# SixLabors/ZlibStream

Measured on AMD Instinct MI355X. Metric: deflate MB/s (input) at level 6, 64 MiB buffers, higher is better.
Workload: dtype u8; 1 GPU; english64: 1 x 67108864-byte pseudo-random-English (Zipf words of alice29.txt) buffer per GPU, level 6, zlib framing, inputs resident in HBM; level=6, buffer_bytes=67108864, buffers_per_gpu=1, compressed_bytes=27425826, parallelism=independent buffers, 1 GPU(s), no collective in the data path

## Files before the change

### zlibstream_amd/csrc/zs_device.h

```cpp
#pragma once
#include <cstddef>
#include "zs_core.h"
#include "zs_lit_engine.h"
#include "zs_fast_sweep.h"
#include "zs_rle.h"

namespace zs {

constexpr int kMatchTile = 16384;
constexpr int kMatchBack = 32512;
constexpr int kMatchFwd = 272;
constexpr int kMatchLdsBytes = kMatchBack + kMatchTile + kMatchFwd;
constexpr int kMatchLdsLinks = kMatchBack + kMatchTile;
constexpr int kMatchLds = kMatchLdsBytes + 2 * kMatchLdsLinks;
constexpr int kAdlerPiece = 65536;

constexpr int64_t kScratchWindow = 0;
constexpr int64_t kScratchHead = 66560;
constexpr int64_t kScratchPrev = kScratchHead + 2 * kHashSize;
constexpr int64_t kScratchHead32 = kScratchPrev + 2 * kWSize;
constexpr int64_t kScratchBytes = kScratchHead32 + 4 * kHashSize;

struct StreamDesc {
    const uint8_t *in;
// ... 78 lines not shown
    uint32_t nsyms;
    int32_t nblocks;
    int64_t out_len;
    uint32_t adler;
    int32_t status;
    int64_t end_bits;
    int32_t r_seg, r_slot, r_kfired, r_kslot;
    uint32_t r_total;
    int32_t r_ncut;
    int32_t r_cut_e[8], r_cut_done[8];
    int32_t deferred, r_scan;
    int32_t r_cutidx;
    int32_t nc[2], cuts_same, cut_diff_idx, cut_diff_pos;
    int32_t poison;
    int32_t spec_run_tiles, spec_ok, spec_wrong;
};
constexpr uint32_t kSpecBail = 1u << 30;
ZS_HD uint32_t spec_pack(int guess, int exit_slot, int count, bool bail) {
    return (uint32_t)guess | ((uint32_t)exit_slot << 9) | ((uint32_t)count << 18) | (bail ? kSpecBail : 0u);
}
ZS_HD int spec_guess(uint32_t r) { return (int)(r & 0x1FF); }
ZS_HD int spec_exit(uint32_t r) { return (int)((r >> 9) & 0x1FF); }
ZS_HD int spec_count(uint32_t r) { return (int)((r >> 18) & 0xFFF); }
constexpr int kSpecMinInput = 1 << 20;
constexpr int kSpecLenBits = 10;
constexpr int kSpecWarm = 128;
constexpr int kSpecRunsDen = 8;
struct K5Spec {
    uint32_t *rec;
    uint32_t *base;
// ... 33 lines not shown
```

### zlibstream_amd/csrc/zs_engine.hip

```cpp
#include <hip/hip_runtime.h>

#include <algorithm>
#include <cstdio>
#include <cstdlib>
#include <cstring>
#include <functional>
#include <string>
#include <thread>
#include <vector>

#define ZS_BUILDING_LIBRARY
#include "../../include/zsgpu.h"
#include "zs_kernels.hip"
#include "zs_inflate_par.hip"
#include "zs_inflate_tok.hip"
#include "zs_png.hip"
#include "zs_crc32.hip"
#include "zs_gzip.hip"
#include "zs_zip.hip"
#include "zs_tiff.hip"
#include "zs_exr.hip"
#include "zs_plan.h"

using namespace zs;

namespace {

struct DevBuf {
    void *p = nullptr;
    size_t cap = 0;
};

enum Stage {
    kStClear, kStAdler, kStLinks, kStMatch, kStChunkMap, kStSegMap, kStResolve, kStExpand, kStEmitSyms, kStTail, kStTrees,
    kStOffsets, kStEmitBits, kStSpecWalk, kStSpecVerify, kStCrc32, kStSpecCompact, kStPngExpand, kStPngSplit, kStPngPack, kStPngSurvey, kStPngCompose, kStPngDiff, kStPngCrop, kStCount
};
const char *const kStageNames[kStCount] = {"clear", "adler", "links", "match", "chunkmap", "segmap", "resolve", "expand",
                                           "emit_syms", "tail", "trees", "offsets", "emit_bits", "spec_walk", "spec_verify", "crc32_frame",
                                           "spec_compact", "png_expand", "png_split", "png_pack", "png_survey", "png_compose", "png_diff", "png_crop"};

enum PngBuf {
    kBufPngImg, kBufPngSeg, kBufPngCtr, kBufPngFimg, kBufPngScratch, kBufPngA7img, kBufPngInflated, kBufPngPasses, kBufCrcDesc, kBufCrcRes, kBufPngZs, kBufPngGather,
    kBufPngXimg, kBufPngRaw, kBufPngSimg, kBufPngSplit, kBufPngGimg, kBufPngVimg, kBufPngVrec, kBufPngPacked, kBufPngCimg, kBufPngFrames, kBufPngDimg, kBufPngDrec,
    kBufPngKimg, kBufPngCrop,
    kBufWrapHead, kBufWrapGather, kBufWrapZs, kBufWrapFiles, kBufZipZs, kBufTiffChunks, kBufTiffDesc, kBufTiffZs, kBufExrChunks, kBufExrDesc, kBufExrZs, kBufExrSegs,
    kBufPngCount
};

struct PlanCache;

}

struct zs_ctx {
    int device = 0;
    hipStream_t stream = nullptr;
    hipStream_t aux = nullptr;
    hipEvent_t ev_fork = nullptr, ev_join = nullptr, ev_pre0 = nullptr, ev_pre = nullptr;
    hipEvent_t ev_spec[4] = {};
    std::string err;
    bool profiling = false;
    int fast_fallbacks = 0;
    int round_runs = 0;
    int cut_rounds = 0;
    int lit_fallbacks = 0;
    int spec_streams = 0, spec_fallbacks = 0, spec_wrong_chunks = 0;
    int spec_periodic = 0;
    int64_t dbg_blk_off = 0, dbg_chunk_off = 0, dbg_nchunks = 0, dbg_spec_n = 0, dbg_n_spec = 0;
    int64_t lit_engine_bytes = 0;
    std::vector<int64_t> inf_used;
    int64_t *inf_probe = nullptr;
    int inf_lane_streams = 0;
    int inf_wave_streams = 0;
    int64_t png_segments = 0;
// ... 97 lines not shown
template <class T>
T *dev(DevBuf &b) {
    return (T *)b.p;
}


struct RunOpts : PlanRun {
    int64_t end_bits = 0;
};

struct LaunchEnv {
    bool no_plan_reuse = getenv("ZS_NO_PLAN_REUSE") != nullptr, no_supmap = getenv("ZS_NO_SUPMAP") != nullptr;
    bool no_defer = getenv("ZS_NO_DEFER") != nullptr, force_rounds = getenv("ZS_FORCE_ROUNDS") != nullptr;
    bool tail_serial = getenv("ZS_TAIL_SERIAL") != nullptr, tail_fork = getenv("ZS_TAIL_FORK") != nullptr, fast_no_probe = getenv("ZS_FAST_NO_PROBE") != nullptr;
    bool no_whole_runs = getenv("ZS_NO_WHOLE_RUNS") != nullptr, whole_runs = getenv("ZS_WHOLE_RUNS") != nullptr;
    bool debug = getenv("ZS_DEBUG") != nullptr, debug_cuts = getenv("ZS_DEBUG_CUTS") != nullptr, debug_fa = getenv("ZS_DEBUG_FA") != nullptr;
    const char *debug_chain = getenv("ZS_DEBUG_CHAIN"), *debug_chain_want = getenv("ZS_DEBUG_CHAIN_WANT");
    int k5_ahead = getenv("ZS_K5_AHEAD") ? atoi(getenv("ZS_K5_AHEAD")) : 1;
    int spec_corrupt = getenv("ZS_SPEC_CORRUPT") ? atoi(getenv("ZS_SPEC_CORRUPT")) : -1;
    static bool host_times() {
        static const bool v = getenv("ZS_HOST_TIMES") != nullptr;
        return v;
    }
    static const char *eb_tiles() {
        static const char *const v = getenv("ZS_EB_TILES");
        return v;
    }
};
struct RoundsEnv {
    int max_rounds = getenv("ZS_FR_MAX_ROUNDS") ? atoi(getenv("ZS_FR_MAX_ROUNDS")) : 0;
// ... 34 lines not shown
    PlanEnv penv = plan_env_read();
    LaunchEnv env;
    FoldedWrites folded;
    PlanArgs pa;
    bool any_writes = false, no_rounds_this_call = false, plan_hit = false, plan_keep = false;
    double ht_plan = 0, ht_launched = 0;
    const StreamDesc *d_sd = nullptr;
    StreamState *d_st = nullptr, *hst = nullptr;
    const uint2 *d_work = nullptr;
    bool prof = false;
    K5Spec k5s{};
    int spec_ok_streams = 0;
    bool need_maps = true, spec_ran = false;
    bool fork_recorded = false;
    bool tail_late = false, tail_serial = false, use_sup = false;
    int defer_mode = 0, cut_stride = 0;
    bool done = false, answer = false;

    double ht_us() const { return std::chrono::duration<double, std::micro>(std::chrono::steady_clock::now() - ht0).count(); }
    const uint2 *work(int list) const { return d_work + lay.work[list]; }
    void mark(int i) {
        if (prof) (void)hipEventRecord(c->ev[i], stream);
    }
    bool rerun(int force_seq_, bool rounds_, const std::vector<uint8_t> *force_lit_) {
        c->lit_engine_bytes -= pl.lit_bytes;
        done = true;
        return answer = run_pipeline(c, n, in, in_len, out, out_cap, out_len, status, level, strategy, hash_variant, stream, writes, force_seq_, ro, rounds_, force_lit_);
    }
    void launch_tail(hipStream_t on) {
        hipLaunchKernelGGL(zs_tail_kernel, dim3((unsigned)n), dim3(1024), kTailLds, on, d_sd, d_st, dev<uint16_t>(c->link),
// ... 431 lines not shown
        for (int s0 = 0; s0 < n; s0 += 65535) launch(dim3((unsigned)((max_tiles + 3) / 4), (unsigned)std::min(n - s0, 65535)), s0);
    };
    tiles([&](dim3 tg, int s0) { hipLaunchKernelGGL(zs_rle_starts_kernel, tg, dim3(256), 0, stream, d_sd, rt, s0); });
    hipLaunchKernelGGL(zs_rle_scan_kernel, dim3((unsigned)n), dim3(1024), 0, stream, d_sd, rt);
    tiles([&](dim3 tg, int s0) {
        hipLaunchKernelGGL(zs_rle_pass_kernel<0>, tg, dim3(256), 0, stream, d_sd, rt, dev<uint32_t>(c->syms), dev<int32_t>(c->blk_end), dev<int32_t>(c->blk_top), s0);
    });
    hipLaunchKernelGGL(zs_rle_sums_kernel, dim3((unsigned)n), dim3(1024), 0, stream, d_sd, d_st, rt);
    tiles([&](dim3 tg, int s0) {
        hipLaunchKernelGGL(zs_rle_pass_kernel<1>, tg, dim3(256), 0, stream, d_sd, rt, dev<uint32_t>(c->syms), dev<int32_t>(c->blk_end), dev<int32_t>(c->blk_top), s0);
    });
    return true;
}

bool DeflateCall::tails_and_symbols() {
    if (!tail_late && !tail_serial) {
        if (!fork_recorded || need_maps) ZS_HIP(c, hipEventRecord(c->ev_fork, stream));
        ZS_HIP(c, hipStreamWaitEvent(c->aux, c->ev_fork, 0));
        launch_tail(c->aux);
        ZS_HIP(c, hipEventRecord(c->ev_join, c->aux));
    }
    if (!pl.w_segs.empty() && need_maps)
        hipLaunchKernelGGL(zs_expand_kernel, dim3((unsigned)((pl.w_segs.size() + 63) / 64)), dim3(64), 0, stream, d_sd, d_st,
                           work(kWSegs), (int)pl.w_segs.size(), dev<uint2>(c->mm), dev<uint16_t>(c->link),
                           dev<uint32_t>(c->maps), dev<uint16_t>(c->seg_entry), dev<uint32_t>(c->seg_symbase),
                           dev<uint8_t>(c->stale), dev<uint16_t>(c->entry), dev<uint32_t>(c->symbase), c->crc_tab, lv, strategy,
                           hash_variant);
    mark(8);
    if (!pl.w_chunks.empty() && need_maps)
        hipLaunchKernelGGL((zs_emit_syms_lane_kernel<4, 0>), dim3((unsigned)((pl.w_chunks.size() + 63) / 64)), dim3(kK5Threads), 0, stream, d_sd, d_st,
                           work(kWChunks), (int)pl.w_chunks.size(), dev<uint2>(c->mm), dev<uint16_t>(c->link), dev<uint16_t>(c->entry),
                           dev<uint32_t>(c->symbase), dev<uint32_t>(c->syms), dev<int32_t>(c->blk_end), dev<int32_t>(c->blk_top),
                           c->crc_tab, lv, strategy, hash_variant, env.k5_ahead, k5s);
    mark(9);
    if (tail_serial) launch_tail(stream);
    else if (!tail_late) ZS_HIP(c, hipStreamWaitEvent(stream, c->ev_join, 0));
    hipLaunchKernelGGL(zs_body_blocks_kernel, dim3((unsigned)n), dim3(256), 0, stream, d_sd, d_st, dev<int32_t>(c->blk_end),
                       dev<int32_t>(c->blk_top), dev<BlockRec>(c->blocks), dev<uint32_t>(c->syms));
    if (tail_late) launch_tail(stream);
    return true;
}

bool DeflateCall::spec_runs() {
    if (!env.fast_no_probe && force_seq == 0 && !pl.any_dual) {
        hipLaunchKernelGGL(zs_fast_probe_kernel, dim3((unsigned)n), dim3(256), 0, stream, d_sd, dev<uint16_t>(c->link), dev<int32_t>(c->run_fail));
        std::vector<int32_t> np((size_t)n, 0);
        ZS_HIP(c, hipMemcpyAsync(np.data(), c->run_fail.p, 4 * (size_t)n, hipMemcpyDeviceToHost, stream));
        ZS_HIP(c, hipStreamSynchronize(stream));
        for (int i = 0; i < n; i++)
            if (np[(size_t)i]) {
                ZS_HIP(c, hipStreamSynchronize(c->aux));
                return rerun(1, false, force_lit);
            }
// ... 40 lines not shown
                       dev<uint32_t>(c->run_syms), dev<FastRunOut>(c->run_outs), dev<uint32_t>(c->syms), dev<int32_t>(c->blk_end),
                       dev<int32_t>(c->blk_top));
    hipLaunchKernelGGL(zs_fast_blocks_kernel, dim3((unsigned)n), dim3(64), 0, stream, d_sd, d_st, dev<FastRunOut>(c->run_outs),
                       dev<int32_t>(c->blk_end), dev<int32_t>(c->blk_top), dev<BlockRec>(c->blocks), n);
    return true;
}

bool DeflateCall::blocks_and_bits() {
    const int trees_threads = pl.w_blocks.size() > 8192 ? 128 : 256;
    if (n >= 64 && !penv.no_live_list) {
        int32_t *const d_live = (int32_t *)((uint8_t *)c->sd.p + lay.sd_bytes);
        hipLaunchKernelGGL(zs_live_scan_kernel, dim3(1), dim3(1024), 0, stream, d_st, n, d_live);
        hipLaunchKernelGGL(zs_live_fill_kernel, dim3((unsigned)((pl.w_blocks.size() + 255) / 256)), dim3(256), 0, stream, d_live, n,
                           (uint32_t)pl.w_blocks.size(), dev<uint2>(c->work) + lay.work[kWBlocks]);
    }
    hipLaunchKernelGGL(zs_trees_kernel, dim3((unsigned)pl.w_blocks.size()), dim3(trees_threads), 0, stream, d_sd, d_st, work(kWBlocks),
                       dev<uint32_t>(c->syms), dev<BlockRec>(c->blocks), dev<TreeWork>(c->trees), dev<BlockInfo>(c->info), dev<int32_t>(c->tile_bits), strategy, level);
    mark(11);
    ZS_HIP(c, hipStreamWaitEvent(stream, c->ev_pre, 0));
    hipLaunchKernelGGL(zs_offsets_kernel, dim3((unsigned)n), dim3(256), 0, stream, d_sd, d_st, dev<BlockRec>(c->blocks),
                       dev<BlockInfo>(c->info), dev<TreeWork>(c->trees), dev<uint32_t>(c->pieces), level, n);
    mark(12);
    int eb_tiles = kEbTiles;
    if (level != 0) {
        int64_t longest = 0;
        for (int i = 0; i < n; i++) longest = std::max(longest, in_len[i]);
        eb_tiles = (int)std::min<int64_t>(kEbTiles, (longest + 1) / kEbTile + 1);
    }
    if (env.eb_tiles()) eb_tiles = std::max(1, std::min(kEbTiles, atoi(env.eb_tiles())));
    hipLaunchKernelGGL(zs_emit_bits_kernel, dim3((unsigned)pl.w_blocks.size(), (unsigned)(1 + eb_tiles)), dim3(256), 0, stream, d_sd, d_st,
                       work(kWBlocks), dev<uint32_t>(c->syms), dev<BlockRec>(c->blocks), dev<TreeWork>(c->trees), dev<BlockInfo>(c->info),
                       dev<int32_t>(c->tile_bits));
    mark(13);
    ZS_HIP(c, hipGetLastError());
    hst = (StreamState *)c->pinned;
    ZS_HIP(c, hipMemcpyAsync(hst, d_st, sizeof(StreamState) * (size_t)n, hipMemcpyDeviceToHost, stream));
    ht_launched = ht_us();
    ZS_HIP(c, hipStreamSynchronize(stream));
    pc.in_flight = false;
    if (pc.valid && !plan_hit) pc.gen = c->plan_gen;
    if (env.host_times())
        fprintf(stderr, "zs: host: plan + uploads %.0f us%s, all launched at %.0f us, device done at %.0f us\n", ht_plan, c->plan_reused ? " (kept plan)" : "", ht_launched,
                ht_us());
    c->last_op = lv.func == 1 ? 2 : 0;
    return true;
}

void DeflateCall::debug_dumps() {
// ... 21 lines not shown
        const size_t nw = wr->ends.size();
        std::vector<int32_t> wb(nw);
        (void)hipMemcpy(wb.data(), pl.sd[0].wr_blk, 4 * nw, hipMemcpyDeviceToHost);
        fprintf(stderr, "[zs] run of %lld bytes, %zu Writes, %d blocks, body ends at %d, resume %d; blocks before each Write:", (long long)in_len[0], nw, hst[0].nblocks,
                pl.sd[0].body_end, pl.sd[0].resume);
        for (size_t k = 0; k < nw && k < 24; k++) fprintf(stderr, " %d(end %lld, flush %d)", wb[k], (long long)wr->ends[k], wr->flush.empty() ? 0 : wr->flush[k]);
        fprintf(stderr, "\n");
    }
}

void DeflateCall::stage_times() {
    for (int i = 0; i < kStCount; i++) {
        float ms = 0;
        if (i >= kStLinks && i <= kStEmitBits) (void)hipEventElapsedTime(&ms, c->ev[i], c->ev[i + 1]);
        c->stage_ms[i] = ms;
    }
    if (spec_ran) {
        float a = 0, b = 0, m = 0;
        (void)hipEventElapsedTime(&a, c->ev[kStChunkMap], c->ev_spec[0]);
        (void)hipEventElapsedTime(&b, c->ev_spec[0], c->ev_spec[1]);
        (void)hipEventElapsedTime(&m, c->ev_spec[1], c->ev[kStChunkMap + 1]);
        c->stage_ms[kStSpecWalk] = a, c->stage_ms[kStSpecVerify] = b, c->stage_ms[kStChunkMap] = m;
        float k = 0;
        (void)hipEventElapsedTime(&k, c->ev_spec[2], c->ev_spec[3]);
        c->stage_ms[kStSpecCompact] = k;
        c->stage_ms[kStSpecVerify] = b > k ? b - k : 0;
    }
}

bool DeflateCall::finish() {
// ... 145 lines not shown
void zs_ctx_destroy(zs_ctx *c);
int zs_ctx_create(int device, zs_ctx **out) {
    if (!out) return ZS_STREAM_ERROR;
    *out = nullptr;
    int count = 0;
    if (hipGetDeviceCount(&count) != hipSuccess || count <= 0 || device < 0 || device >= count) return ZS_STREAM_ERROR;
    if (hipSetDevice(device) != hipSuccess) return ZS_STREAM_ERROR;
    zs_ctx *c = new zs_ctx();
    c->device = device;
    if (hipStreamCreateWithFlags(&c->stream, hipStreamNonBlocking) != hipSuccess) {
        zs_ctx_destroy(c);
        return ZS_MEM_ERROR;
    }
    for (auto &e : c->ev) (void)hipEventCreate(&e);
    for (auto &e : c->ev_spec) (void)hipEventCreate(&e);
    for (auto &e : c->ev_png) (void)hipEventCreate(&e);
    {
        int *d_ok = nullptr, ok = 0;
        if (hipMalloc((void **)&d_ok, sizeof(int)) != hipSuccess) {
            zs_ctx_destroy(c);
            return ZS_MEM_ERROR;
        }
        hipLaunchKernelGGL(zs_lds_order_kernel, dim3(1), dim3(64), 0, c->stream, d_ok);
        const bool copied = hipMemcpyAsync(&ok, d_ok, sizeof(int), hipMemcpyDeviceToHost, c->stream) == hipSuccess &&
                            hipStreamSynchronize(c->stream) == hipSuccess;
        (void)hipFree(d_ok);
        if (!copied || !ok) {
            fprintf(stderr, "zsgpu: LDS lane-order self-test failed on device %d; this build cannot run there\n", device);
            zs_ctx_destroy(c);
            return ZS_STREAM_ERROR;
        }
    }
    if (hipStreamCreateWithFlags(&c->aux, hipStreamNonBlocking) != hipSuccess ||
        hipEventCreateWithFlags(&c->ev_fork, hipEventDisableTiming) != hipSuccess ||
        hipEventCreateWithFlags(&c->ev_join, hipEventDisableTiming) != hipSuccess ||
        hipEventCreateWithFlags(&c->ev_pre0, hipEventDisableTiming) != hipSuccess ||
        hipEventCreateWithFlags(&c->ev_pre, hipEventDisableTiming) != hipSuccess ||
        hipEventCreateWithFlags(&c->ev_verdict, hipEventDisableTiming) != hipSuccess) {
        zs_ctx_destroy(c);
        return ZS_MEM_ERROR;
    }
    std::vector<uint32_t> tab(1024);
    for (int t = 0; t < 4; t++)
        for (int i = 0; i < 256; i++) tab[(size_t)t * 256 + i] = crc32c_table_entry(t, (uint32_t)i);
    if (hipMalloc((void **)&c->crc_tab, 4096) != hipSuccess ||
        hipMemcpy(c->crc_tab, tab.data(), 4096, hipMemcpyHostToDevice) != hipSuccess ||
        hipFuncSetAttribute((const void *)zs_match_kernel, hipFuncAttributeMaxDynamicSharedMemorySize, kMatchLds + 16) != hipSuccess ||
        hipFuncSetAttribute((const void *)zs_resolve_kernel, hipFuncAttributeMaxDynamicSharedMemorySize, kResolveLds) != hipSuccess ||
        hipFuncSetAttribute((const void *)zs_links_kernel, hipFuncAttributeMaxDynamicSharedMemorySize, kLkLds) != hipSuccess ||
        hipFuncSetAttribute((const void *)zs_tail_kernel, hipFuncAttributeMaxDynamicSharedMemorySize, kTailLds) != hipSuccess ||
        hipFuncSetAttribute((const void *)zs_fast_run_kernel, hipFuncAttributeMaxDynamicSharedMemorySize, kFastRunLds) != hipSuccess ||
        hipFuncSetAttribute((const void *)zs_fast_sweep_kernel<1024, kFsTile1, false>, hipFuncAttributeMaxDynamicSharedMemorySize, (fs_lds_bytes<1024, kFsTile1>())) != hipSuccess ||
// ... 36 lines not shown
        if (e) (void)hipEventDestroy(e);
    if (c->pinned) (void)hipHostFree(c->pinned);
    if (c->plan_pin) (void)hipHostFree(c->plan_pin);
    delete c->plan;
    if (c->ev_verdict) (void)hipEventDestroy(c->ev_verdict);
    if (c->pin_io) (void)hipHostFree(c->pin_io);
    if (c->pin_out) (void)hipHostFree(c->pin_out);
    for (auto &e : c->ev)
        if (e) (void)hipEventDestroy(e);
    for (auto &e : c->ev_spec)
        if (e) (void)hipEventDestroy(e);
    if (c->ev_fork) (void)hipEventDestroy(c->ev_fork);
    if (c->ev_join) (void)hipEventDestroy(c->ev_join);
    if (c->ev_pre0) (void)hipEventDestroy(c->ev_pre0);
    if (c->ev_pre) (void)hipEventDestroy(c->ev_pre);
    if (c->aux) (void)hipStreamDestroy(c->aux);
    if (c->stream) (void)hipStreamDestroy(c->stream);
    delete c;
}

const char *zs_ctx_last_error(const zs_ctx *c) { return c ? c->err.c_str() : "no context"; }

int64_t zs_deflate_bound(int64_t n) { return n + (n >> 3) + 1024; }

void zs_ctx_set_profiling(zs_ctx *c, int enable) {
    if (c) c->profiling = enable != 0;
}
int zs_ctx_stage_count(const zs_ctx *) { return kStCount; }
int64_t zs_ctx_counter(const zs_ctx *c, const char *name) {
    if (!c || !name) return -1;
// ... 29 lines not shown
        memcpy(out, state, sizeof state);
        return sizeof state;
    }
    if (k == "blk_end") src = dev<int32_t>(c->blk_end) + c->dbg_blk_off, bytes = 4 * (int64_t)(ss.body_syms / kBlockSyms);
    else if (k == "blk_top") src = dev<int32_t>(c->blk_top) + c->dbg_blk_off, bytes = 4 * (int64_t)(ss.body_syms / kBlockSyms);
    else if (k == "symbase") src = dev<uint32_t>(c->symbase) + c->dbg_chunk_off, bytes = 4 * c->dbg_nchunks;
    else if (k == "spec_base") src = dev<uint32_t>(c->spec_rec) + c->dbg_n_spec, bytes = 4 * c->dbg_spec_n;
    else return -1;
    if (bytes > cap || (bytes > 0 && !src)) return -1;
    if (bytes > 0 && hipMemcpy(out, src, (size_t)bytes, hipMemcpyDeviceToHost) != hipSuccess) return -1;
    return bytes;
}

const char *zs_ctx_stage_name(const zs_ctx *c, int s) {
    static const char *const inf_names[6] = {"inf_find", "inf_measure", "inf_chain", "inf_decode", "inf_windows", "inf_resolve"};
    if (s == kStCrc32 || s == kStSpecCompact || s == kStPngExpand || s == kStPngSplit || s == kStPngPack || s == kStPngSurvey || s == kStPngCompose || s == kStPngDiff || s == kStPngCrop) return kStageNames[s];
    if (c && c->last_op == 1) return s >= 0 && s < 6 ? inf_names[s] : "";
    if (c && c->last_op == 2 && s == kStExpand) return "fast_sweep";
    if (c && c->last_op == 2 && s == kStTail) return "fast_runs+tail";
    return s >= 0 && s < kStCount ? kStageNames[s] : "";
}
double zs_ctx_stage_ms(const zs_ctx *c, int s) { return c && s >= 0 && s < kStCount ? c->stage_ms[s] : 0.0; }

int zs_deflate_batch_device(zs_ctx *c, int n, const void *const *in, const int64_t *in_len, void *const *out,
                            const int64_t *out_cap, int64_t *out_len, int *status, int level, int strategy, int hash_variant,
                            void *hip_stream) {
    if (!check_args(c, n, in_len, level, strategy)) return ZS_STREAM_ERROR;
    if (n == 0) return ZS_OK;
    if (hipSetDevice(c->device) != hipSuccess) return ZS_STREAM_ERROR;
    hipStream_t s = hip_stream ? (hipStream_t)hip_stream : c->stream;
    int rc = ZS_OK;
// ... 746 lines not shown
```

### zlibstream_amd/csrc/zs_kernels.hip

```cpp
#include <hip/hip_runtime.h>

#include <type_traits>

#include "zs_device.h"
#include "zs_png.h"

namespace zs {

typedef uint32_t __attribute__((aligned(1))) u32u;
typedef uint64_t __attribute__((aligned(1))) u64u;
typedef const __attribute__((address_space(1))) uint8_t *gcbytes;
typedef __attribute__((address_space(1))) uint8_t *gbytes_w;
__device__ __forceinline__ gcbytes as_global(const uint8_t *p) { return (gcbytes)(uintptr_t)p; }
__device__ __forceinline__ gbytes_w as_global(uint8_t *p) { return (gbytes_w)(uintptr_t)p; }
typedef const __attribute__((address_space(1))) uint32_t __attribute__((aligned(1))) *gcu32u;
typedef const __attribute__((address_space(1))) uint64_t __attribute__((aligned(1))) *gcu64u;
__device__ __forceinline__ uint32_t g_u32_bytes(gcbytes p) {
    return (uint32_t)p[0] | ((uint32_t)p[1] << 8) | ((uint32_t)p[2] << 16) | ((uint32_t)p[3] << 24);
}
typedef uint32_t u32x4 __attribute__((ext_vector_type(4)));
typedef const __attribute__((address_space(1))) u32x4 *gcu32x4;
__device__ __forceinline__ uint32_t lds_u32(const uint8_t *base, int idx) {
    const uint32_t *q = (const uint32_t *)(base + (idx & ~3));
    return __builtin_amdgcn_alignbyte(q[1], q[0], (uint32_t)idx & 3u);
// ... 1977 lines not shown
        out[i] = v;
        before += i < cut ? sym_len(v) : 0;
    }
    if (cut < 0) return;
#pragma unroll
    for (int d = 32; d >= 1; d >>= 1) before += __shfl_xor(before, d, 64);
    if (lane != 0) return;
    const ChunkCtx cx = spec_chunk_ctx(s, c, sp.len_bits);
    const int64_t start = spec_first_start(cx.cs, spec_guess(r)) + before;
    const bool odd = cx.m != 0 && slab[sp.stride - 1] == (uint32_t)cut;
    const uint32_t bi = (base + (uint32_t)cut) / kBlockSyms;
    blk_end[s.blk_off + bi] = (int32_t)spec_sym_end(start, slab[cut]);
    blk_top[s.blk_off + bi] = (int32_t)spec_sym_top(start, odd);
}

__global__ __launch_bounds__(256) void zs_body_blocks_kernel(const StreamDesc *sd, const StreamState *st, const int32_t *blk_end,
                                                             const int32_t *blk_top, BlockRec *blocks, uint32_t *syms) {
    const StreamDesc s = sd[blockIdx.x];
    if (s.fast_runs > 0 || st[blockIdx.x].deferred) return;
    if (s.resume)
        for (uint32_t i = threadIdx.x; i < s.start_syms; i += blockDim.x) syms[s.sym_off + i] = s.persist->syms[i];
    const int nb_body = (int)(st[blockIdx.x].body_syms / kBlockSyms);
    BlockRec *blk = blocks + s.blk_off;
    for (int i = threadIdx.x; i < nb_body; i += blockDim.x) {
        int64_t start = i ? blk_end[s.blk_off + i - 1] : (s.resume ? s.start_block : 0);
        int64_t end = blk_end[s.blk_off + i];
        BlockRec r;
        r.start = start;
        r.sym_start = (int64_t)i * kBlockSyms;
        r.stored_len = (int32_t)(end - start);
        r.nsyms = kBlockSyms;
        r.can_store = start >= s.base0 + (int64_t)kWSize * (s.rle_end >= 0 ? rle_refills_fired_at(blk_top[s.blk_off + i], s.kl)
                                                                            : refills_fired_at(blk_top[s.blk_off + i] - s.base0, s.kl));
        r.eof = 0;
        blk[i] = r;
    }
    if (s.wr_blk && s.wr_end && s.n_wr > 1) {
        const StreamState &ss = st[blockIdx.x];
        const int64_t read_to = s.nsegs > 0 ? (int64_t)s.seg_after[ss.k_done] : 0;
        for (int w = 1 + (int)threadIdx.x; w < s.n_wr; w += blockDim.x) {
            if (s.wr_end[w - 1] >= read_to) continue;
            const int64_t bound = s.wr_end[w - 1] - (kMinLookahead - 1);
            int lo = 0, hi = nb_body;
            while (lo < hi) {
                const int mid = (lo + hi) >> 1;
                if ((int64_t)blk_top[s.blk_off + mid] < bound) lo = mid + 1;
                else hi = mid;
            }
            s.wr_blk[w] = lo;
        }
    }
// ... 711 lines not shown
        if (live_pre[mid] <= (int32_t)g) lo = mid;
        else hi = mid - 1;
    }
    work[g] = make_uint2((uint32_t)lo, g - (uint32_t)live_pre[lo]);
}

#ifdef ZS_BS_PROF
#define BS_PF(i) { const long long now_ = wall_clock64(); pf[i] += now_ - pf_t; pf_t = now_; }
#else
#define BS_PF(i)
#endif
typedef u32x4 __attribute__((aligned(4))) u32x4a4;
typedef u32x4 __attribute__((aligned(8))) u32x4a8;
__global__ __launch_bounds__(256) void zs_trees_kernel(const StreamDesc *sd, const StreamState *st, const uint2 *work,
                                                       const uint32_t *syms, const BlockRec *blocks, TreeWork *trees,
                                                       BlockInfo *info, int32_t *tile_bits, int strategy, int level) {
    __shared__ __attribute__((aligned(16))) TreeWork tw;
    __shared__ SideTree sw;
    __shared__ uint32_t hl[kLCodes], hd[kDCodes];
    __shared__ uint32_t hk[kHeapSize + 8];
    __shared__ uint32_t pd[kHeapSize + 1], nc[16];
    __shared__ uint32_t hk2[SideTree::kHeap + 8], pd2[SideTree::kHeap + 1], nc2[16];
    __shared__ uint32_t sh_tile[2 * kEbTiles];
    __shared__ int sh_type;
#ifdef ZS_BS_PROF
    long long pf[8] = {0, 0, 0, 0, 0, 0, 0, 0}, pf_t = wall_clock64();
#endif
    uint2 w = work[blockIdx.x];
    if (w.x == kNoWork || st[w.x].deferred) return;
    const StreamDesc s = sd[w.x];
    const int b = (int)w.y;
    if (b >= st[w.x].nblocks) return;
    const BlockRec r = blocks[s.blk_off + b];
    if (level == 0 && r.nsyms == 0 && s.plan_nblk > 0) {
        if (threadIdx.x == 0) {
            BlockInfo bi;
            bi.type = r.can_store ? 0 : 1;
            bi.bits = r.can_store ? 0 : 10;
            bi.bit_start = 0;
            info[s.blk_off + b] = bi;
        }
        return;
    }
    const int tid = (int)threadIdx.x, nthr = (int)blockDim.x, lane = tid & 63, wave = tid >> 6;
    for (int i = tid; i < kLCodes; i += nthr) hl[i] = 0;
    for (int i = tid; i < kDCodes; i += nthr) hd[i] = 0;
    if (tid < 2 * kEbTiles) sh_tile[tid] = 0;
// ... 146 lines not shown
    if (w0) atomicOr(w, w0);
    if (w1) atomicOr(w + 1, w1);
    if (w2) atomicOr(w + 2, w2);
}
struct OrBitsAt {
    uint8_t *out;
    int64_t cap;
    int64_t bit_base;
    __device__ void operator()(int64_t pos, uint32_t v, int nbits) const {
        pos -= bit_base;
        if ((pos >> 3) + 12 <= cap) or_bits(out, pos, v, nbits);
    }
};
__global__ __launch_bounds__(256) void zs_offsets_kernel(const StreamDesc *sd, StreamState *st, const BlockRec *blocks,
                                                         BlockInfo *info, const TreeWork *trees, const uint32_t *adler_pieces,
                                                         int level, int nstreams) {
    __shared__ int32_t sh_type[1024], sh_bits[1024], sh_len[1024], sh_eof[1024];
    __shared__ int64_t sh_start[1024];
    __shared__ uint32_t ad_v[256];
    __shared__ uint64_t ad_len[256];
    __shared__ int64_t sh_pos, sh_wsum[4];
    __shared__ int sh_bad;
    FlushAcct fa;
    int fa_w = 0;
    const bool flushing = sd[blockIdx.x].wr_flush != nullptr;
    const int si = blockIdx.x;
    if (st[si].deferred) return;
    const StreamDesc s = sd[si];
    StreamState &ss = st[si];
    const int nb = ss.nblocks;
    LitPersist *ps = s.persist;
    const int64_t start_bits = s.cont_bits ? ps->fa.bits : 16;
    const int64_t bit_base = s.cont_bits ? (start_bits & ~7LL) : 0;
    if (threadIdx.x == 0) sh_pos = start_bits, sh_bad = 0;
    const OrBitsAt fa_put{s.out, s.out_cap, bit_base};
    if (flushing) {
        if (s.cont_bits) fa = ps->fa;
        else fa_init(fa, s.out_chunk, level, s.raw != 0);
        if (!s.mid_write) fa_enter(fa);
    }
    if (threadIdx.x == 0 && s.cont_bits && s.out_cap > 0) s.out[0] = (uint8_t)s.carry_byte;
    __syncthreads();
    for (int b0 = 0; b0 < nb; b0 += 1024) {
        int cnt = nb - b0 < 1024 ? nb - b0 : 1024;
        for (int i = threadIdx.x; i < cnt; i += 256) {
            const BlockInfo bi = info[s.blk_off + b0 + i];
            const BlockRec r = blocks[s.blk_off + b0 + i];
            sh_type[i] = bi.type, sh_bits[i] = bi.bits, sh_len[i] = r.stored_len, sh_eof[i] = r.eof;
        }
        __syncthreads();
        int irregular = 0;
        for (int i = threadIdx.x; i < cnt; i += 256) irregular |= (sh_type[i] == 0) || (sh_eof[i] && i != cnt - 1);
        irregular = __syncthreads_or(irregular | (int)flushing);
        if (!irregular) {
            const int lane = threadIdx.x & 63, wave = threadIdx.x >> 6;
            int64_t b4[4], mine = 0;
            for (int k = 0; k < 4; k++) {
                const int i = threadIdx.x * 4 + k;
// ... 39 lines not shown
                if (flushing) {
                    fa.bits = pos;
                    fa.last_eob_len = sh_type[i] == 0 ? 8 : sh_type[i] == 1 ? 7 : trees[s.blk_off + b0 + i].ltree[kEndBlock].dl;
                    const int f = sh_eof[i] >> 1;
                    if (f) fa_end_of_write(fa, f, fa_put);
                    else fa_after_block(fa);
                    pos = fa.bits;
                }
            }
            sh_pos = pos;
        }
        __syncthreads();
        for (int i = threadIdx.x; i < cnt; i += 256) info[s.blk_off + b0 + i].bit_start = sh_start[i] - bit_base;
        __syncthreads();
    }
    uint32_t acc = 1;
    uint64_t acc_len = 0;
    {
        const int per = (s.n_adler + 255) / 256;
        for (int k = 0; k < per; k++) {
            int i = threadIdx.x * per + k;
            if (i >= s.n_adler) break;
            int64_t len = (int64_t)s.n - (int64_t)i * kAdlerPiece;
            if (len > kAdlerPiece) len = kAdlerPiece;
            acc = adler_combine(acc, adler_pieces[s.adler_off + i], (uint64_t)len);
            acc_len += (uint64_t)len;
        }
        ad_v[threadIdx.x] = acc, ad_len[threadIdx.x] = acc_len;
    }
    __syncthreads();
// ... 15 lines not shown
        ss.out_len = bytes;
        ss.status = sh_bad ? -2 : (bytes + 8 > s.out_cap ? -5 : 0);
        return;
    }
    int64_t total = (pos - bit_base) / 8 + 4;
    ss.out_len = total;
    if (sh_bad) {
        ss.status = -2;
        return;
    }
    if (total > s.out_cap) {
        ss.status = -5;
        return;
    }
    ss.status = 0;
    if (!s.cont_bits) {
        unsigned hdr = zlib_header(level);
        s.out[0] = (uint8_t)(hdr >> 8);
        s.out[1] = (uint8_t)hdr;
    }
    uint8_t *t = s.out + (pos - bit_base) / 8;
    t[0] = (uint8_t)(ad >> 24), t[1] = (uint8_t)(ad >> 16), t[2] = (uint8_t)(ad >> 8), t[3] = (uint8_t)ad;
}

struct OrPut {
    uint8_t *out;
    int64_t pos;
    __device__ void operator()(unsigned value, int nbits) {
        or_bits(out, pos, value, nbits);
        pos += nbits;
    }
// ... 19 lines not shown
        const uint32_t w0 = (uint32_t)lo, w1 = (uint32_t)(lo >> 32), w2 = sh ? (uint32_t)(v >> (64 - sh)) : 0;
        if (w0) atomicOr(&w[k], w0);
        if (w1) atomicOr(&w[k + 1], w1);
        if (w2) atomicOr(&w[k + 2], w2);
        pos += (uint32_t)nbits;
    }
    __device__ void operator()(unsigned value, int nbits) { put64(value, nbits); }
};
#ifdef ZS_BS_PROF
#define BS_PF(i) { const long long now_ = wall_clock64(); pf[i] += now_ - pf_t; pf_t = now_; }
#else
#define BS_PF(i)
#endif
__global__ __launch_bounds__(256) void zs_emit_bits_kernel(const StreamDesc *sd, const StreamState *st, const uint2 *work,
                                                           const uint32_t *syms, const BlockRec *blocks, const TreeWork *trees,
                                                           const BlockInfo *info, const int32_t *tile_bits) {
    __shared__ uint32_t lt[kLCodes], dt[kDCodes];
    __shared__ uint32_t obuf[kEbWords];
    __shared__ uint32_t wsum[4];
    __shared__ uint32_t sh_bits;
#ifdef ZS_BS_PROF
    long long pf[4] = {0, 0, 0, 0}, pf_t = wall_clock64();
#endif
    uint2 w = work[blockIdx.x];
    if (w.x == kNoWork || st[w.x].deferred) return;
    const StreamDesc s = sd[w.x];
    const int b = (int)w.y;
    if (b >= st[w.x].nblocks || st[w.x].status != 0) return;
    const BlockRec r = blocks[s.blk_off + b];
    const BlockInfo bi = info[s.blk_off + b];
    uint8_t *out = s.out;
    const int tid = threadIdx.x, lane = lane_id(), wave = tid >> 6;
    const int part = (int)blockIdx.y, ntl = (int)gridDim.y - 1;
    if (bi.type == 0) {
        int64_t pos = bi.bit_start;
        int64_t byte = (pos + 3 + 7) >> 3;
        if (part == 0 && tid == 0) {
            or_bits(out, pos, (uint64_t)(r.eof & 1), 3);
            unsigned len = (unsigned)r.stored_len;
            out[byte] = (uint8_t)len, out[byte + 1] = (uint8_t)(len >> 8);
            out[byte + 2] = (uint8_t)~len, out[byte + 3] = (uint8_t)(~len >> 8);
        }
        const gcbytes src = as_global(s.in) + (r.start - s.abs_off);
        const gbytes_w dst = as_global(out) + byte + 4;
        typedef u32x4 __attribute__((aligned(1))) u32x4u;
// ... 367 lines not shown
```

Baseline: 15870 MB/s.

## Split deflate backend into body and tail parts overlapped across two streams

```diff
diff --git a/zlibstream_amd/csrc/zs_device.h b/zlibstream_amd/csrc/zs_device.h
--- a/zlibstream_amd/csrc/zs_device.h
+++ b/zlibstream_amd/csrc/zs_device.h
@@ -116,6 +116,8 @@
     int32_t nc[2], cuts_same, cut_diff_idx, cut_diff_pos;
     int32_t poison;
     int32_t spec_run_tiles, spec_ok, spec_wrong;
+    int32_t body_bad;
+    int64_t body_bits;
 };
 constexpr uint32_t kSpecBail = 1u << 30;
 ZS_HD uint32_t spec_pack(int guess, int exit_slot, int count, bool bail) {
diff --git a/zlibstream_amd/csrc/zs_engine.hip b/zlibstream_amd/csrc/zs_engine.hip
--- a/zlibstream_amd/csrc/zs_engine.hip
+++ b/zlibstream_amd/csrc/zs_engine.hip
@@ -33,11 +33,11 @@
 
 enum Stage {
     kStClear, kStAdler, kStLinks, kStMatch, kStChunkMap, kStSegMap, kStResolve, kStExpand, kStEmitSyms, kStTail, kStTrees,
-    kStOffsets, kStEmitBits, kStSpecWalk, kStSpecVerify, kStCrc32, kStSpecCompact, kStPngExpand, kStPngSplit, kStPngPack, kStPngSurvey, kStPngCompose, kStPngDiff, kStPngCrop, kStCount
+    kStOffsets, kStEmitBits, kStSpecWalk, kStSpecVerify, kStCrc32, kStSpecCompact, kStPngExpand, kStPngSplit, kStPngPack, kStPngSurvey, kStPngCompose, kStPngDiff, kStPngCrop, kStPart1, kStCount
 };
 const char *const kStageNames[kStCount] = {"clear", "adler", "links", "match", "chunkmap", "segmap", "resolve", "expand",
                                            "emit_syms", "tail", "trees", "offsets", "emit_bits", "spec_walk", "spec_verify", "crc32_frame",
-                                           "spec_compact", "png_expand", "png_split", "png_pack", "png_survey", "png_compose", "png_diff", "png_crop"};
+                                           "spec_compact", "png_expand", "png_split", "png_pack", "png_survey", "png_compose", "png_diff", "png_crop", "part1_chain"};
 
 enum PngBuf {
     kBufPngImg, kBufPngSeg, kBufPngCtr, kBufPngFimg, kBufPngScratch, kBufPngA7img, kBufPngInflated, kBufPngPasses, kBufCrcDesc, kBufCrcRes, kBufPngZs, kBufPngGather,
@@ -57,6 +57,7 @@
     hipStream_t aux = nullptr;
     hipEvent_t ev_fork = nullptr, ev_join = nullptr, ev_pre0 = nullptr, ev_pre = nullptr;
     hipEvent_t ev_spec[4] = {};
+    hipEvent_t ev_syms = nullptr, ev_part0 = nullptr, ev_part1[2] = {};
     std::string err;
     bool profiling = false;
     int fast_fallbacks = 0;
@@ -184,6 +185,7 @@
     bool no_defer = getenv("ZS_NO_DEFER") != nullptr, force_rounds = getenv("ZS_FORCE_ROUNDS") != nullptr;
     bool tail_serial = getenv("ZS_TAIL_SERIAL") != nullptr, tail_fork = getenv("ZS_TAIL_FORK") != nullptr, fast_no_probe = getenv("ZS_FAST_NO_PROBE") != nullptr;
     bool no_whole_runs = getenv("ZS_NO_WHOLE_RUNS") != nullptr, whole_runs = getenv("ZS_WHOLE_RUNS") != nullptr;
+    bool no_split_backend = getenv("ZS_NO_SPLIT_BACKEND") != nullptr;
     bool debug = getenv("ZS_DEBUG") != nullptr, debug_cuts = getenv("ZS_DEBUG_CUTS") != nullptr, debug_fa = getenv("ZS_DEBUG_FA") != nullptr;
     const char *debug_chain = getenv("ZS_DEBUG_CHAIN"), *debug_chain_want = getenv("ZS_DEBUG_CHAIN_WANT");
     int k5_ahead = getenv("ZS_K5_AHEAD") ? atoi(getenv("ZS_K5_AHEAD")) : 1;
@@ -248,6 +250,7 @@
     bool need_maps = true, spec_ran = false;
     bool fork_recorded = false;
     bool tail_late = false, tail_serial = false, use_sup = false;
+    bool split = false;
     int defer_mode = 0, cut_stride = 0;
     bool done = false, answer = false;
 
@@ -709,11 +712,18 @@
 }
 
 bool DeflateCall::tails_and_symbols() {
+    const bool beside_k5 = need_maps && (!pl.w_segs.empty() || !pl.w_chunks.empty());
+    if (!tail_late && !tail_serial && (n < 64 || penv.no_live_list) && !env.no_split_backend && pl.n_runs == 0 && !beside_k5) {
+        int64_t longest = 0;
+        for (int i = 0; i < n; i++) longest = std::max(longest, in_len[i]);
+        split = longest >= kBlockSyms;
+    }
     if (!tail_late && !tail_serial) {
         if (!fork_recorded || need_maps) ZS_HIP(c, hipEventRecord(c->ev_fork, stream));
         ZS_HIP(c, hipStreamWaitEvent(c->aux, c->ev_fork, 0));
         launch_tail(c->aux);
-        ZS_HIP(c, hipEventRecord(c->ev_join, c->aux));
+        if (split && prof) (void)hipEventRecord(c->ev_part1[0], c->aux);
+        if (!split) ZS_HIP(c, hipEventRecord(c->ev_join, c->aux));
     }
     if (!pl.w_segs.empty() && need_maps)
         hipLaunchKernelGGL(zs_expand_kernel, dim3((unsigned)((pl.w_segs.size() + 63) / 64)), dim3(64), 0, stream, d_sd, d_st,
@@ -728,10 +738,20 @@
                            dev<uint32_t>(c->symbase), dev<uint32_t>(c->syms), dev<int32_t>(c->blk_end), dev<int32_t>(c->blk_top),
                            c->crc_tab, lv, strategy, hash_variant, env.k5_ahead, k5s);
     mark(9);
+    auto body_blocks = [&](hipStream_t on, int part) {
+        hipLaunchKernelGGL(zs_body_blocks_kernel, dim3((unsigned)n), dim3(256), 0, on, d_sd, d_st, dev<int32_t>(c->blk_end),
+                           dev<int32_t>(c->blk_top), dev<BlockRec>(c->blocks), dev<uint32_t>(c->syms), part);
+    };
+    if (split) {
+        ZS_HIP(c, hipEventRecord(c->ev_syms, stream));
+        body_blocks(stream, kPartBody);
+        ZS_HIP(c, hipStreamWaitEvent(c->aux, c->ev_syms, 0));
+        body_blocks(c->aux, kPartRest);
+        return true;
+    }
     if (tail_serial) launch_tail(stream);
     else if (!tail_late) ZS_HIP(c, hipStreamWaitEvent(stream, c->ev_join, 0));
-    hipLaunchKernelGGL(zs_body_blocks_kernel, dim3((unsigned)n), dim3(256), 0, stream, d_sd, d_st, dev<int32_t>(c->blk_end),
-                       dev<int32_t>(c->blk_top), dev<BlockRec>(c->blocks), dev<uint32_t>(c->syms));
+    body_blocks(stream, kPartAll);
     if (tail_late) launch_tail(stream);
     return true;
 }
@@ -802,13 +822,20 @@
         hipLaunchKernelGGL(zs_live_fill_kernel, dim3((unsigned)((pl.w_blocks.size() + 255) / 256)), dim3(256), 0, stream, d_live, n,
                            (uint32_t)pl.w_blocks.size(), dev<uint2>(c->work) + lay.work[kWBlocks]);
     }
-    hipLaunchKernelGGL(zs_trees_kernel, dim3((unsigned)pl.w_blocks.size()), dim3(trees_threads), 0, stream, d_sd, d_st, work(kWBlocks),
-                       dev<uint32_t>(c->syms), dev<BlockRec>(c->blocks), dev<TreeWork>(c->trees), dev<BlockInfo>(c->info), dev<int32_t>(c->tile_bits), strategy, level);
+    auto trees = [&](hipStream_t on, int part) {
+        hipLaunchKernelGGL(zs_trees_kernel, dim3((unsigned)pl.w_blocks.size()), dim3(trees_threads), 0, on, d_sd, d_st, work(kWBlocks), dev<uint32_t>(c->syms),
+                           dev<BlockRec>(c->blocks), dev<TreeWork>(c->trees), dev<BlockInfo>(c->info), dev<int32_t>(c->tile_bits), strategy, level, part);
+    };
+    auto offsets = [&](hipStream_t on, int part) {
+        hipLaunchKernelGGL(zs_offsets_kernel, dim3((unsigned)n), dim3(256), 0, on, d_sd, d_st, dev<BlockRec>(c->blocks), dev<BlockInfo>(c->info),
+                           dev<TreeWork>(c->trees), dev<uint32_t>(c->pieces), level, n, part);
+    };
+    trees(stream, split ? kPartBody : kPartAll);
     mark(11);
     ZS_HIP(c, hipStreamWaitEvent(stream, c->ev_pre, 0));
-    hipLaunchKernelGGL(zs_offsets_kernel, dim3((unsigned)n), dim3(256), 0, stream, d_sd, d_st, dev<BlockRec>(c->blocks),
-                       dev<BlockInfo>(c->info), dev<TreeWork>(c->trees), dev<uint32_t>(c->pieces), level, n);
+    offsets(stream, split ? kPartBody : kPartAll);
     mark(12);
+    if (split) ZS_HIP(c, hipEventRecord(c->ev_part0, stream));
     int eb_tiles = kEbTiles;
     if (level != 0) {
         int64_t longest = 0;
@@ -816,10 +843,21 @@
         eb_tiles = (int)std::min<int64_t>(kEbTiles, (longest + 1) / kEbTile + 1);
     }
     if (env.eb_tiles()) eb_tiles = std::max(1, std::min(kEbTiles, atoi(env.eb_tiles())));
-    hipLaunchKernelGGL(zs_emit_bits_kernel, dim3((unsigned)pl.w_blocks.size(), (unsigned)(1 + eb_tiles)), dim3(256), 0, stream, d_sd, d_st,
-                       work(kWBlocks), dev<uint32_t>(c->syms), dev<BlockRec>(c->blocks), dev<TreeWork>(c->trees), dev<BlockInfo>(c->info),
-                       dev<int32_t>(c->tile_bits));
+    auto emit_bits = [&](hipStream_t on, int part) {
+        hipLaunchKernelGGL(zs_emit_bits_kernel, dim3((unsigned)pl.w_blocks.size(), (unsigned)(1 + eb_tiles)), dim3(256), 0, on, d_sd, d_st, work(kWBlocks),
+                           dev<uint32_t>(c->syms), dev<BlockRec>(c->blocks), dev<TreeWork>(c->trees), dev<BlockInfo>(c->info), dev<int32_t>(c->tile_bits), part);
+    };
+    emit_bits(stream, split ? kPartBody : kPartAll);
     mark(13);
+    if (split) {
+        trees(c->aux, kPartRest);
+        ZS_HIP(c, hipStreamWaitEvent(c->aux, c->ev_part0, 0));
+        offsets(c->aux, kPartRest);
+        emit_bits(c->aux, kPartRest);
+        if (prof) (void)hipEventRecord(c->ev_part1[1], c->aux);
+        ZS_HIP(c, hipEventRecord(c->ev_join, c->aux));
+        ZS_HIP(c, hipStreamWaitEvent(stream, c->ev_join, 0));
+    }
     ZS_HIP(c, hipGetLastError());
     hst = (StreamState *)c->pinned;
     ZS_HIP(c, hipMemcpyAsync(hst, d_st, sizeof(StreamState) * (size_t)n, hipMemcpyDeviceToHost, stream));
@@ -871,6 +909,11 @@
         float ms = 0;
         if (i >= kStLinks && i <= kStEmitBits) (void)hipEventElapsedTime(&ms, c->ev[i], c->ev[i + 1]);
         c->stage_ms[i] = ms;
+    }
+    if (split) {
+        float p1 = 0;
+        (void)hipEventElapsedTime(&p1, c->ev_part1[0], c->ev_part1[1]);
+        c->stage_ms[kStPart1] = p1;
     }
     if (spec_ran) {
         float a = 0, b = 0, m = 0;
@@ -1046,6 +1089,7 @@
     }
     for (auto &e : c->ev) (void)hipEventCreate(&e);
     for (auto &e : c->ev_spec) (void)hipEventCreate(&e);
+    for (auto &e : c->ev_part1) (void)hipEventCreate(&e);
     for (auto &e : c->ev_png) (void)hipEventCreate(&e);
     {
         int *d_ok = nullptr, ok = 0;
@@ -1068,6 +1112,8 @@
         hipEventCreateWithFlags(&c->ev_join, hipEventDisableTiming) != hipSuccess ||
         hipEventCreateWithFlags(&c->ev_pre0, hipEventDisableTiming) != hipSuccess ||
         hipEventCreateWithFlags(&c->ev_pre, hipEventDisableTiming) != hipSuccess ||
+        hipEventCreateWithFlags(&c->ev_syms, hipEventDisableTiming) != hipSuccess ||
+        hipEventCreateWithFlags(&c->ev_part0, hipEventDisableTiming) != hipSuccess ||
         hipEventCreateWithFlags(&c->ev_verdict, hipEventDisableTiming) != hipSuccess) {
         zs_ctx_destroy(c);
         return ZS_MEM_ERROR;
@@ -1134,6 +1180,10 @@
     if (c->ev_join) (void)hipEventDestroy(c->ev_join);
     if (c->ev_pre0) (void)hipEventDestroy(c->ev_pre0);
     if (c->ev_pre) (void)hipEventDestroy(c->ev_pre);
+    if (c->ev_syms) (void)hipEventDestroy(c->ev_syms);
+    if (c->ev_part0) (void)hipEventDestroy(c->ev_part0);
+    for (auto &e : c->ev_part1)
+        if (e) (void)hipEventDestroy(e);
     if (c->aux) (void)hipStreamDestroy(c->aux);
     if (c->stream) (void)hipStreamDestroy(c->stream);
     delete c;
@@ -1193,7 +1243,7 @@
 
 const char *zs_ctx_stage_name(const zs_ctx *c, int s) {
     static const char *const inf_names[6] = {"inf_find", "inf_measure", "inf_chain", "inf_decode", "inf_windows", "inf_resolve"};
-    if (s == kStCrc32 || s == kStSpecCompact || s == kStPngExpand || s == kStPngSplit || s == kStPngPack || s == kStPngSurvey || s == kStPngCompose || s == kStPngDiff || s == kStPngCrop) return kStageNames[s];
+    if (s == kStCrc32 || s == kStSpecCompact || s == kStPngExpand || s == kStPngSplit || s == kStPngPack || s == kStPngSurvey || s == kStPngCompose || s == kStPngDiff || s == kStPngCrop || s == kStPart1) return kStageNames[s];
     if (c && c->last_op == 1) return s >= 0 && s < 6 ? inf_names[s] : "";
     if (c && c->last_op == 2 && s == kStExpand) return "fast_sweep";
     if (c && c->last_op == 2 && s == kStTail) return "fast_runs+tail";
diff --git a/zlibstream_amd/csrc/zs_kernels.hip b/zlibstream_amd/csrc/zs_kernels.hip
--- a/zlibstream_amd/csrc/zs_kernels.hip
+++ b/zlibstream_amd/csrc/zs_kernels.hip
@@ -2015,15 +2015,25 @@
     blk_top[s.blk_off + bi] = (int32_t)spec_sym_top(start, odd);
 }
 
+enum { kPartAll = -1, kPartBody = 0, kPartRest = 1 };
+__device__ __forceinline__ int stream_body_blocks(int part, const StreamDesc &s, const StreamState &ss) {
+    if (part == kPartAll) return 0;
+    const bool splits = s.wr_flush == nullptr && s.n_wr <= 1 && s.final_run && !s.resume && !s.cont && !s.cont_bits && s.fast_runs == 0 &&
+                        s.plan_nblk == 0 && !ss.deferred;
+    return splits ? (int)(ss.body_syms / kBlockSyms) : 0;
+}
+
 __global__ __launch_bounds__(256) void zs_body_blocks_kernel(const StreamDesc *sd, const StreamState *st, const int32_t *blk_end,
-                                                             const int32_t *blk_top, BlockRec *blocks, uint32_t *syms) {
+                                                             const int32_t *blk_top, BlockRec *blocks, uint32_t *syms, int part) {
     const StreamDesc s = sd[blockIdx.x];
     if (s.fast_runs > 0 || st[blockIdx.x].deferred) return;
+    const int nb0 = stream_body_blocks(part, s, st[blockIdx.x]);
+    if (part == kPartBody && nb0 == 0) return;
     if (s.resume)
         for (uint32_t i = threadIdx.x; i < s.start_syms; i += blockDim.x) syms[s.sym_off + i] = s.persist->syms[i];
     const int nb_body = (int)(st[blockIdx.x].body_syms / kBlockSyms);
     BlockRec *blk = blocks + s.blk_off;
-    for (int i = threadIdx.x; i < nb_body; i += blockDim.x) {
+    for (int i = threadIdx.x; i < (part == kPartRest && nb0 > 0 ? 0 : nb_body); i += blockDim.x) {
         int64_t start = i ? blk_end[s.blk_off + i - 1] : (s.resume ? s.start_block : 0);
         int64_t end = blk_end[s.blk_off + i];
         BlockRec r;
@@ -2036,6 +2046,7 @@
         r.eof = 0;
         blk[i] = r;
     }
+    if (part == kPartBody) return;
     if (s.wr_blk && s.wr_end && s.n_wr > 1) {
         const StreamState &ss = st[blockIdx.x];
         const int64_t read_to = s.nsegs > 0 ? (int64_t)s.seg_after[ss.k_done] : 0;
@@ -2777,7 +2788,7 @@
 typedef u32x4 __attribute__((aligned(8))) u32x4a8;
 __global__ __launch_bounds__(256) void zs_trees_kernel(const StreamDesc *sd, const StreamState *st, const uint2 *work,
                                                        const uint32_t *syms, const BlockRec *blocks, TreeWork *trees,
-                                                       BlockInfo *info, int32_t *tile_bits, int strategy, int level) {
+                                                       BlockInfo *info, int32_t *tile_bits, int strategy, int level, int part) {
     __shared__ __attribute__((aligned(16))) TreeWork tw;
     __shared__ SideTree sw;
     __shared__ uint32_t hl[kLCodes], hd[kDCodes];
@@ -2793,7 +2804,8 @@
     if (w.x == kNoWork || st[w.x].deferred) return;
     const StreamDesc s = sd[w.x];
     const int b = (int)w.y;
-    if (b >= st[w.x].nblocks) return;
+    const int nb0 = stream_body_blocks(part, s, st[w.x]);
+    if (part == kPartBody ? b >= nb0 : (b < nb0 || b >= st[w.x].nblocks)) return;
     const BlockRec r = blocks[s.blk_off + b];
     if (level == 0 && r.nsyms == 0 && s.plan_nblk > 0) {
         if (threadIdx.x == 0) {
@@ -2970,7 +2982,7 @@
 };
 __global__ __launch_bounds__(256) void zs_offsets_kernel(const StreamDesc *sd, StreamState *st, const BlockRec *blocks,
                                                          BlockInfo *info, const TreeWork *trees, const uint32_t *adler_pieces,
-                                                         int level, int nstreams) {
+                                                         int level, int nstreams, int part) {
     __shared__ int32_t sh_type[1024], sh_bits[1024], sh_len[1024], sh_eof[1024];
     __shared__ int64_t sh_start[1024];
     __shared__ uint32_t ad_v[256];
@@ -2984,11 +2996,14 @@
     if (st[si].deferred) return;
     const StreamDesc s = sd[si];
     StreamState &ss = st[si];
-    const int nb = ss.nblocks;
+    const int nb0 = stream_body_blocks(part, s, ss);
+    if (part == kPartBody && nb0 == 0) return;
+    const int nb = part == kPartBody ? nb0 : ss.nblocks;
+    const int nb_first = part == kPartBody ? 0 : nb0;
     LitPersist *ps = s.persist;
-    const int64_t start_bits = s.cont_bits ? ps->fa.bits : 16;
+    const int64_t start_bits = s.cont_bits ? ps->fa.bits : nb_first > 0 ? ss.body_bits : 16;
     const int64_t bit_base = s.cont_bits ? (start_bits & ~7LL) : 0;
-    if (threadIdx.x == 0) sh_pos = start_bits, sh_bad = 0;
+    if (threadIdx.x == 0) sh_pos = start_bits, sh_bad = nb_first > 0 ? ss.body_bad : 0;
     const OrBitsAt fa_put{s.out, s.out_cap, bit_base};
     if (flushing) {
         if (s.cont_bits) fa = ps->fa;
@@ -2997,7 +3012,7 @@
     }
     if (threadIdx.x == 0 && s.cont_bits && s.out_cap > 0) s.out[0] = (uint8_t)s.carry_byte;
     __syncthreads();
-    for (int b0 = 0; b0 < nb; b0 += 1024) {
+    for (int b0 = nb_first; b0 < nb; b0 += 1024) {
         int cnt = nb - b0 < 1024 ? nb - b0 : 1024;
         for (int i = threadIdx.x; i < cnt; i += 256) {
             const BlockInfo bi = info[s.blk_off + b0 + i];
@@ -3067,6 +3082,17 @@
         for (int i = threadIdx.x; i < cnt; i += 256) info[s.blk_off + b0 + i].bit_start = sh_start[i] - bit_base;
         __syncthreads();
     }
+    if (part == kPartBody) {
+        if (threadIdx.x == 0) {
+            ss.body_bits = sh_pos, ss.body_bad = sh_bad;
+            if (s.out_cap >= 2) {
+                const unsigned hdr = zlib_header(level);
+                s.out[0] = (uint8_t)(hdr >> 8);
+                s.out[1] = (uint8_t)hdr;
+            }
+        }
+        return;
+    }
     uint32_t acc = 1;
     uint64_t acc_len = 0;
     {
@@ -3112,7 +3138,7 @@
         return;
     }
     ss.status = 0;
-    if (!s.cont_bits) {
+    if (!s.cont_bits && nb_first == 0) {
         unsigned hdr = zlib_header(level);
         s.out[0] = (uint8_t)(hdr >> 8);
         s.out[1] = (uint8_t)hdr;
@@ -3162,7 +3188,7 @@
 #endif
 __global__ __launch_bounds__(256) void zs_emit_bits_kernel(const StreamDesc *sd, const StreamState *st, const uint2 *work,
                                                            const uint32_t *syms, const BlockRec *blocks, const TreeWork *trees,
-                                                           const BlockInfo *info, const int32_t *tile_bits) {
+                                                           const BlockInfo *info, const int32_t *tile_bits, int split_part) {
     __shared__ uint32_t lt[kLCodes], dt[kDCodes];
     __shared__ uint32_t obuf[kEbWords];
     __shared__ uint32_t wsum[4];
@@ -3174,9 +3200,15 @@
     if (w.x == kNoWork || st[w.x].deferred) return;
     const StreamDesc s = sd[w.x];
     const int b = (int)w.y;
-    if (b >= st[w.x].nblocks || st[w.x].status != 0) return;
+    const int nb0 = stream_body_blocks(split_part, s, st[w.x]);
+    if (split_part == kPartBody ? b >= nb0 : (b >= st[w.x].nblocks || st[w.x].status != 0)) return;
     const BlockRec r = blocks[s.blk_off + b];
     const BlockInfo bi = info[s.blk_off + b];
+    if (b < nb0) {
+        const int64_t end_byte = bi.type == 0 ? ((bi.bit_start + 3 + 7) >> 3) + 4 + r.stored_len : (bi.bit_start + bi.bits + 7) >> 3;
+        const bool fits = end_byte + 12 <= s.out_cap;
+        if (fits != (split_part == kPartBody)) return;
+    }
     uint8_t *out = s.out;
     const int tid = threadIdx.x, lane = lane_id(), wave = tid >> 6;
     const int part = (int)blockIdx.y, ntl = (int)gridDim.y - 1;
```

Measured after the change: 16440 MB/s (median of 6 runs). +3.6%, better.
